# julesser/crocoddyl

Measured on AMD Instinct MI355X. Metric: FDDP iterations/sec + MPC solves/sec, Talos contact T=100, batch=1024, higher is better.
Workload: dtype f64

## Files before the change

### crocoddyl_amd/_abi.py

```python
import ctypes as C

ABI_VERSION = 3

FDDP_OK = 0
FDDP_ERR_INVALID_ARG = -1
FDDP_ERR_RUNTIME = -2
FDDP_ERR_UNSUPPORTED = -3
FDDP_ERR_NO_DEVICE = -4
FDDP_ERR_CALLBACK_ABORT = -5

STATUS_RUNNING, STATUS_CONVERGED, STATUS_REGMAX = 0, 1, 2

KNOT_LQR, KNOT_UNICYCLE, KNOT_EULER_DIFFLQR, KNOT_EULER_FREEFWD, KNOT_EULER_CONTACTFWD, KNOT_IMPULSEFWD = 1, 2, 3, 4, 5, 6
PARAM_HEADER = 4

Q_FX, Q_FU, Q_LXX, Q_LXU, Q_LUU, Q_LX, Q_LU, Q_XNEXT, Q_FS, Q_K, Q_KV = range(11)
Q_COST = 19
Q_VXX, Q_VX, Q_QXX, Q_QXU, Q_QUU, Q_QX, Q_QU = range(11, 18)
Q_QUU_INV = 18

SOLVER_FDDP, SOLVER_BOXFDDP = 0, 1

MB_W2, MB_W1, MB_X2, MB_X8, MB_S2 = range(5)
FWD_GENERIC, FWD_FAST, FWD_MB, FWD_MB2 = range(4)
# ... 83 lines not shown
    "get_x0": (C.c_int, [P, D]),
    "get_params": (C.c_int, [P, C.POINTER(Params)]),
    "get_xs": (C.c_int, [P, D, C.c_int]),
    "get_us": (C.c_int, [P, D, C.c_int]),
    "get_xs_try": (C.c_int, [P, D]),
    "get_us_try": (C.c_int, [P, D]),
    "set_debug": (C.c_int, [P, C.c_int]),
    "synchronize": (C.c_int, [P]),
    "get_stream": (C.c_int, [P, C.POINTER(P)]),
    "get_timing": (C.c_int, [P, D, C.POINTER(C.c_int64)]),
    "set_timing": (C.c_int, [P, C.c_int]),
    "device_bytes": (C.c_int64, [P]),
    "get_solver_kind": (C.c_int, [P, I32]),
    "set_callback": (C.c_int, [P, IterationCallback, C.c_void_p]),
    "get_line_search_info": (C.c_int, [P, I32, I32]),
    "get_kernel_info": (C.c_int, [P, I32]),
    "boxqp_default_params": (None, [C.POINTER(BoxQPParams)]),
    "boxqp_solve": (C.c_int, [C.c_int, C.c_int, C.c_int, D, D, D, D, D, C.POINTER(BoxQPParams), D, U64, U64, D, I32]),
}


def bind(lib, prefix, protos):
    for name, (res, args) in protos.items():
        fn = getattr(lib, prefix + name)
        fn.restype = res
        fn.argtypes = args


def dptr(a):
    if a is None:
# ... 3 lines not shown
```

### crocoddyl_amd/csrc/fddp_device.hpp

```cpp
#pragma once

#include <hip/hip_runtime.h>
#include <stdint.h>

#include "../../include/fddp_hip.h"

namespace fddp {

__host__ __device__ inline bool is_mb_kind(int kind) {
  return kind == FDDP_KNOT_EULER_FREEFWD || kind == FDDP_KNOT_EULER_CONTACTFWD || kind == FDDP_KNOT_IMPULSEFWD;
}

constexpr int kWave = 64;

struct ElemState {
  double cost;
  double cost_try;
  double stop;
  double xreg, ureg;
  double steplength;
  double dV, dVexp;
  double dg, dq, dv;
  double d0, d1;
  int32_t is_feasible, was_feasible;
  int32_t recalc;
  int32_t iter;
  int32_t status;
  int32_t active;
// ... 266 lines not shown
```

### crocoddyl_amd/csrc/fddp_hip.hip

```cpp
#define FDDP_TU_MAIN 1
#include <hip/hip_runtime.h>

#include <algorithm>
#include <cmath>
#include <cstdio>
#include <cstdlib>
#include <cstring>
#include <string>
#include <vector>

#include "../../include/fddp_hip.h"
#include "fddp_device.hpp"
#include "fddp_kernels.hpp"
#include "fast_path.hpp"
#include "bwd_mfma.hpp"
#include "ktab.hpp"
#include "launch_plan.hpp"

using namespace fddp;
using plan::block_doubles;
using plan::mb_block_check;

namespace fddp {
namespace ktab {
// ... 124 lines not shown
  o.mb_spill = env_int("FDDP_MB_SPILL", -1);
  o.fwd_mb_off = is0("FDDP_FWD_MB");
  o.fwd_mbw = env_int("FDDP_FWD_MBW", 0);
  if (const char* ew = env("FDDP_BWD_WAVES")) o.bwd_waves = ew[0] == '1' ? 1 : (ew[0] == '4' ? 4 : 8);
  o.bwd_generic = env("FDDP_BACKWARD") && std::strcmp(env("FDDP_BACKWARD"), "generic") == 0;
  o.fast_off = is0("FDDP_FAST");
  if (prev)
    o.ls_par = prev->ls_par;
  else if (env("CROCODDYL_AMD_LS_PAR"))
    o.ls_par = std::max(1, std::min(16, env_int("CROCODDYL_AMD_LS_PAR", 0)));
  return o;
}

}

struct fddp_handle_s {
  fddp_dims dims;
  int device = 0;
  int cus = 0;
  plan::LaunchPlan plan;
  int npar_alloc = 1;
  bool npar_chosen = false;
  hipStream_t stream = nullptr;
  std::vector<fddp_knot_desc> knots;
  int64_t n_params = 0;
  int64_t params_cap = 0;
  fddp_params prm;
  Dev D;
  std::vector<void*> allocs;
  double* staging = nullptr;
  int64_t staging_len = 0;
  double* d_out = nullptr;
  int* d_count = nullptr;
  int* h_count = nullptr;
  bool debug = false;
  double* dbg[7] = {nullptr, nullptr, nullptr, nullptr, nullptr, nullptr, nullptr};
  double* dqi = nullptr;
// ... 172 lines not shown
    KLAUNCH(ktab::backward_mfma(h->plan.var.bwd, dim3(D.B), h->stream, D, to_prm(h->prm), mode));
  else
    KLAUNCH(ktab::backward_generic(dim3(D.B), h->bwd_smem, h->stream, D, to_prm(h->prm), mode));
  return FDDP_OK;
}

static int ensure_par_slots(fddp_handle* h) {
  Dev& D = h->D;
  if (D.npar <= h->npar_alloc) return FDDP_OK;
  const int64_t B = D.B, K1 = D.T + 1, K0 = D.T, q = D.npar - 1;
  int rc;
  double* done = nullptr;
  if ((rc = dalloc(h, &D.pxs, q * B * K1 * D.sX)) || (rc = dalloc(h, &D.pus, q * B * K0 * D.sM)) ||
      (rc = dalloc(h, &D.pxnext, q * B * K0 * D.sX)) || (rc = dalloc(h, &D.pkcost, q * B * K1)) ||
      (rc = dalloc(h, &D.pdvp, q * B * K1)) || (rc = dalloc(h, &D.ptrial, B * D.npar * 4)) ||
      (rc = dalloc(h, &done, (B + 1) / 2)))
    return rc;
  D.ls_done = (int*)done;
  h->npar_alloc = D.npar;
  return FDDP_OK;
}

static void choose_npar(fddp_handle* h, const std::vector<ElemState>& st) {
  if (!h->plan.lds.npar_adapt || h->plan.lds.fast) return;
  const int na = h->prm.n_alphas;
  std::vector<int> t;
  t.reserve(st.size());
  for (const ElemState& s : st) {
    if (s.n_iter_run <= 0) continue;
    int k = na;
    for (int a = 0; a < na; ++a)
      if (s.steplength == h->prm.alphas[a]) {
        k = a + 1;
        break;
      }
    t.push_back(k);
  }
  if (t.empty()) return;
  const double S = h->plan.var.ls_slots;
  double best = 0.;
  int best_g = 1;
  for (int g : {1, 2, 4}) {
    double time = 0.;
    if (g == 1) {
      double w = 0.;
      int tmax = 0;
      for (int v : t) w += v, tmax = std::max(tmax, v);
      time = std::max(std::ceil(w / S), (double)tmax);
    } else {
      for (int k0 = 0; k0 < na; k0 += g) {
        const int slots = std::min(g, na - k0);
        double u = 0.;
        for (int v : t) u += v > k0 ? slots : 0;
        if (u > 0.) time += std::ceil(u / S);
      }
    }
    if (g == 1 || time < best) best = time, best_g = g;
  }
  h->D.npar = best_g;
  h->npar_chosen = true;
}

static int update_ls_order(fddp_handle* h, const std::vector<ElemState>& st) {
  Dev& D = h->D;
  const int B = D.B, na = h->prm.n_alphas;
  if (B < 2 || h->plan.lds.fast) return FDDP_OK;
  if (!D.ls_order) {
    double* p = nullptr;
    int rc;
    if ((rc = dalloc(h, &p, (B + 1) / 2))) return rc;
    D.ls_order = (const int*)p;
  }
  std::vector<int> key(B);
  for (int b = 0; b < B; ++b) {
    const ElemState& s = st[b];
    int k = 0;
    if (s.n_iter_run > 0) {
      k = na;
      for (int a = 0; a < na; ++a)
        if (s.steplength == h->prm.alphas[a]) {
          k = a + 1;
          break;
        }
    }
    key[b] = k;
  }
  h->h_order.resize(B);
  for (int b = 0; b < B; ++b) h->h_order[b] = b;
  std::stable_sort(h->h_order.begin(), h->h_order.end(), [&](int x, int y) { return key[x] > key[y]; });
  HIP_TRY(hipMemcpyAsync((void*)D.ls_order, h->h_order.data(), sizeof(int) * B, hipMemcpyHostToDevice, h->stream));
  return FDDP_OK;
}

int launch_forward(fddp_handle* h, int mode, double alpha, int* count) {
  Timed tm(h, 3);
  const Dev& D = h->D;
  if (!h->plan.lds.fast && mode == 0 && D.npar > 1) {
    int rc;
    if ((rc = ensure_par_slots(h))) return rc;
    const int na = h->prm.n_alphas, G = (na + D.npar - 1) / D.npar;
    h->ls_npar_last = D.npar;
    h->ls_launches_last = G;
    const int v = h->plan.var.fwd;
    for (int g = 0; g < G; ++g) {
      KLAUNCH(ktab::forward(v, dim3(D.B, D.npar), h->plan.lds.fwd_smem, h->stream, D, to_prm(h->prm), 2, 1., nullptr, h->plan.lds.pcap,
                            g));
      KLAUNCH(ktab::ls_select(dim3(D.B), h->stream, D, to_prm(h->prm), g, g == G - 1 ? 1 : 0, count));
    }
    return FDDP_OK;
  }
  if (mode == 0) {
// ... 98 lines not shown

int apply_knots(fddp_handle* h, const fddp_knot_desc* knots, const double* params, int64_t n_params) {
  Dev& D = h->D;
  const fddp_dims& d = h->dims;
  const int64_t K1 = (int64_t)d.T + 1;
  int rc;
  h->knots.assign(knots, knots + K1);
  plan::LaunchPlan& P = h->plan;
  P.ov = read_overrides(&P.ov);
  P.lds = plan::plan_lds(d, knots, params, n_params, P.ov);
  const plan::LdsPlan& L = P.lds;
  D.mbw = L.mbw;
  D.mbw_fwd = L.mbw_fwd;
  D.mbspill = L.mbspill;
  D.mbd = L.mbd;
  if (!(h->npar_chosen && L.has_mb && !P.ov.ls_par)) D.npar = L.npar;
  if (L.error) return fail(FDDP_ERR_INVALID_ARG, L.error);
  D.dxv_mbw = L.dxv_mbw;
  if (n_params > h->params_cap) {
    double* p = nullptr;
    if ((rc = dalloc(h, &p, n_params))) return rc;
    D.params = p;
    h->params_cap = n_params;
  }
  h->n_params = n_params;
  HIP_TRY(hipMemcpyAsync((void*)D.params, params, sizeof(double) * n_params, hipMemcpyHostToDevice, h->stream));
  if (!D.knots) {
    fddp_knot_desc* kd = nullptr;
    if ((rc = dalloc(h, (double**)&kd, (sizeof(fddp_knot_desc) * K1 + 7) / 8))) return rc;
    D.knots = kd;
  }
// ... 186 lines not shown
    return bail(fail(FDDP_ERR_RUNTIME, "hipHostMalloc"));

  std::vector<ElemState> st0(B);
  for (auto& s : st0) {
    std::memset(&s, 0, sizeof(s));
    s.xreg = NAN;
    s.ureg = NAN;
    s.steplength = 1.;
  }
  if (hipMemcpyAsync(D.st, st0.data(), sizeof(ElemState) * B, hipMemcpyHostToDevice, h->stream) != hipSuccess)
    return bail(fail(FDDP_ERR_RUNTIME, "upload state"));
  if ((rc = apply_knots(h, knots, params, n_params))) return bail(rc);
  if (const char* e = std::getenv("FDDP_STAMPS")) {
    if (e[0] == '1') {
      double* p2 = nullptr;
      if ((rc = dalloc(h, &p2, (int64_t)d.B * 140))) return bail(rc);
      D.stamps = (unsigned long long*)p2;
    }
  }
  if (hipStreamSynchronize(h->stream) != hipSuccess) return bail(fail(FDDP_ERR_RUNTIME, "sync after create"));
  *out = h;
  return FDDP_OK;
}

void fddp_destroy(fddp_handle* h) {
  if (!h) return;
  DeviceGuard g(h->device);
  if (h->stream) (void)hipStreamSynchronize(h->stream);
  if (h->D.stamps) {
    std::vector<unsigned long long> v((size_t)h->dims.B * 140);
    if (hipMemcpy(v.data(), h->D.stamps, v.size() * 8, hipMemcpyDeviceToHost) == hipSuccess) {
      const char* names[8] = {"p1_G", "p1_H", "p1_inv", "b1_dma", "p2_K", "p2_Vupd", "b2_p3", "b3_wait"};
      std::fprintf(stderr, "[fddp stamps] mean cycles per element (variant %d):\n", h->plan.var.bwd);
      for (int w = 0; w < h->plan.var.bwd % 10; ++w) {
        std::fprintf(stderr, "  wave %d:", w);
        for (int ph = 0; ph < 8; ++ph) {
          double s2 = 0;
          for (int b = 0; b < h->dims.B; ++b) s2 += (double)v[((size_t)b * 8 + w) * 8 + ph];
          std::fprintf(stderr, " %s=%.0f", names[ph], s2 / h->dims.B);
        }
        std::fprintf(stderr, "\n");
      }
      if (h->plan.lds.has_mb || h->plan.lds.fast) {
        const char* mn[5] = {"state", "params", "gains", "calc", "stores_checks"};
        std::fprintf(stderr, "[fddp stamps] %s rollout, wave 0's mean cycles per element (all trials):",
// ... 2 lines not shown
          double s2 = 0;
          for (int b = 0; b < h->dims.B; ++b) s2 += (double)v[(size_t)h->dims.B * 128 + (size_t)b * 8 + ph];
          std::fprintf(stderr, " %s=%.0f", mn[ph], s2 / h->dims.B);
        }
        std::fprintf(stderr, "\n");
      }
      {
        struct Ev {
          unsigned long long t;
          int d;
        };
        std::vector<std::pair<unsigned long long, std::vector<Ev>>> cus;
        std::vector<std::pair<unsigned long long, std::vector<Ev>>>* pc = &cus;
        unsigned long long t0 = ~0ull, t1 = 0;
        int n = 0;
        for (int b = 0; b < h->dims.B; ++b) {
          const unsigned long long* r = &v[(size_t)h->dims.B * 136 + (size_t)b * 4];
          if (r[0] == 0 || r[2] == 0) continue;
          const unsigned long long hw = r[1];
          const unsigned long long key = ((hw >> 32) << 16) | ((hw >> 8) & 0xff);
          size_t i = 0;
          while (i < pc->size() && (*pc)[i].first != key) ++i;
          if (i == pc->size()) pc->push_back({key, {}});
          (*pc)[i].second.push_back({r[0], 1});
          (*pc)[i].second.push_back({r[2], -1});
          t0 = std::min(t0, r[0]);
          t1 = std::max(t1, r[2]);
          ++n;
        }
        int most = 0;
        double area = 0.;
// ... 190 lines not shown
        if (out) std::copy(cbres.begin(), cbres.end(), out);
        return fail(FDDP_ERR_CALLBACK_ABORT, "fddp_solve: stopped by the iteration callback at iteration " +
                                                 std::to_string(it));
      }
    }
    if (it + 1 < maxiter) {
      HIP_TRY(hipMemcpyAsync(h->h_count, h->d_count, sizeof(int), hipMemcpyDeviceToHost, h->stream));
      HIP_TRY(hipStreamSynchronize(h->stream));
      if (*h->h_count == 0) break;
    }
  }
  if (out) {
    std::vector<ElemState> st;
    if ((rc = download_states(h, st))) return rc;
    for (int b = 0; b < D.B; ++b) fill_result(st[b], &out[b]);
    choose_npar(h, st);
    if ((rc = update_ls_order(h, st))) return rc;
  } else {
    HIP_TRY(hipStreamSynchronize(h->stream));
  }
  if (D.box_stats) {
    unsigned long long bs[4];
    HIP_TRY(hipMemcpy(bs, D.box_stats, sizeof(bs), hipMemcpyDeviceToHost));
    fprintf(stderr, "fddp box stats: %llu QPs, %.3f Newton iterations and %.3f inverses per QP\n", bs[0],
            bs[0] ? (double)bs[1] / bs[0] : 0., bs[0] ? (double)bs[2] / bs[0] : 0.);
  }
  return FDDP_OK;
}

int fddp_get_kernel_info(fddp_handle* h, int32_t out[8]) {
  if (!h || !out) return fail(FDDP_ERR_INVALID_ARG, "fddp_get_kernel_info: null argument");
  DeviceGuard g(h->device);
  out[0] = h->plan.var.mb;
  out[1] = h->plan.var.fwd;
  out[2] = h->plan.var.bwd;
  out[3] = h->D.mbspill;
  out[4] = (int32_t)h->plan.lds.mb_diff_smem;
  out[5] = (int32_t)(h->plan.lds.fast ? h->plan.lds.fwd_fast_smem : h->plan.lds.fwd_smem);
  out[6] = h->D.npar;
  out[7] = 0;
  return FDDP_OK;
}

int fddp_get_line_search_info(fddp_handle* h, int* group_size, int* launches) {
  if (!h) return fail(FDDP_ERR_INVALID_ARG, "fddp_get_line_search_info: null handle");
  if (group_size) *group_size = h->ls_npar_last;
  if (launches) *launches = h->ls_launches_last;
  return FDDP_OK;
}

int fddp_set_callback(fddp_handle* h, fddp_iteration_callback cb, void* user) {
  if (!h) return fail(FDDP_ERR_INVALID_ARG, "fddp_set_callback: null handle");
  if (h->in_solve) return fail(FDDP_ERR_INVALID_ARG, "fddp_set_callback: not from inside a callback");
  h->cb = cb;
  h->cb_user = cb ? user : nullptr;
  return FDDP_OK;
}

int fddp_get_results(fddp_handle* h, fddp_result* out) {
  if (!h || !out) return fail(FDDP_ERR_INVALID_ARG, "fddp_get_results: null");
  DeviceGuard g(h->device);
  std::vector<ElemState> st;
// ... 429 lines not shown
```

### crocoddyl_amd/csrc/fddp_kernels.hpp

```cpp
#pragma once

#include "fddp_device.hpp"
#include "box_qp.hpp"
#include "knots.hpp"

namespace fddp {


__device__ inline int64_t block_doubles_dev(int kind, int nx, int nu, const double* g = nullptr) {
  if (is_mb_kind(kind)) return (int64_t)g[3];
  if (kind == FDDP_KNOT_LQR) return FDDP_PARAM_HEADER + 2LL * nx * nx + 2LL * nx * nu + (int64_t)nu * nu + 2LL * nx + nu;
  if (kind == FDDP_KNOT_UNICYCLE) return FDDP_PARAM_HEADER;
  const int64_t nq = nx / 2;
  return FDDP_PARAM_HEADER + 2 * nq * nq + nq * nu + nq + (int64_t)nx * nx + (int64_t)nx * nu + (int64_t)nu * nu + nx +
         nu;
}

template <int NT>
__device__ __forceinline__ void state_diff_wg(const Dev& D, const double* x0, const double* x1, double* out,
                                              int first = 0) {
  const int n = D.n;
  if (D.nx == n) {
    for (int i = threadIdx.x; i < n; i += NT) out[i] = x1[i] - x0[i];
    return;
// ... 836 lines not shown
    s.iter += 1;
  }
}

#ifndef FDDP_FWD_WPE
#define FDDP_FWD_WPE 2
#endif
#ifndef FDDP_FWD_WPE_MB
#define FDDP_FWD_WPE_MB 3
#endif
template <int NT, bool FAST, bool MB = false, int MBW = FDDP_FWD_WPE_MB>
__global__ __launch_bounds__(NT) __attribute__((amdgpu_waves_per_eu(MB ? MBW : FAST ? FDDP_FWD_WPE : 1))) void forward_kernel(Dev D, Prm prm, int mode, double alpha1, int* active_count,
                                                     int64_t pcap, int group = 0) {
  const int b = D.ls_order ? D.ls_order[blockIdx.x] : (int)blockIdx.x;
  ElemState* st = D.st + b;
  if (mode != 1 && !st->active) return;
  const int slot = mode == 2 ? (int)blockIdx.y : 0;
  const int a2 = group * D.npar + slot;
  if (mode == 2 && (D.ls_done[b] || a2 >= prm.n_alphas)) return;
  extern __shared__ __attribute__((aligned(16))) double sm[];
  double* pl = sm;
  const double* cached = nullptr;
  double *xv, *uv, *xn, *red, *dxv = nullptr, *pa = nullptr, *pdyn = nullptr;
  int* flag;
  if (FAST) {
    xv = pl + pcap;
    uv = xv + D.sX;
    dxv = xv + D.sX + D.sM;
    xn = dxv + D.sN;
    pa = xn + D.sX;
    pdyn = pa + NT;
    red = pdyn + NT;
    flag = (int*)(red + 24);
  } else {
    xv = pl + pcap;
    uv = xv + D.sX;
    xn = uv + D.sM;
    red = xn + D.sX;
    flag = (int*)(red + 5 * (NT / kWave) + 8);
  }
  __shared__ ElemState ss;
  if (threadIdx.x == 0) ss = *st;
#ifdef FDDP_STAMPS_BUILD
  unsigned long long* rs = D.stamps && slot == 0 ? D.stamps + (int64_t)D.B * 136 + (int64_t)b * 4 : nullptr;
  if (rs && threadIdx.x == 0) {
    rs[0] = __builtin_amdgcn_s_memrealtime();
    rs[1] = (unsigned long long)(unsigned)__builtin_amdgcn_s_getreg(4 | (31 << 11)) |
            ((unsigned long long)(unsigned)__builtin_amdgcn_s_getreg(20 | (31 << 11)) << 32);
  }
#endif
  __syncthreads();
  int nwr = D.T + 1;
  double* const mbw = (double*)flag + 2 + (D.dxv_mbw ? 0 : 2 * D.sN);
  double* const dxv_ = D.dxv_mbw ? mbw + D.mbw_fwd - 2 * D.sN : (double*)flag + 2;
  auto trial = [&](double alpha, double& ct, double& dv) {
    if constexpr (FAST)
      return fwd_trial_fast<NT, true>(D, b, ss, alpha, xv, dxv, xn, pa, pdyn, red, flag, ct, dv, pl, pcap, cached);
    else
      return fwd_trial<NT, MB>(D, b, ss, alpha, xv, uv, xn, red, flag, ct, dv, pl, pcap, cached, mbw, dxv_, slot, &nwr);
  };
  bool accepted = false;
  const int na = mode == 0 ? prm.n_alphas : 1;
  for (int a = 0; a < na; ++a) {
    const double alpha = mode == 1 ? alpha1 : prm.alphas[mode == 2 ? a2 : a];
    double ct, dv;
    bool ok;
    [[clang::always_inline]] ok = trial(alpha, ct, dv);
    if (mode == 1) {
      if (threadIdx.x == 0) {
        st->fwd_fail = ok ? 0 : 1;
        st->cost_try = ct;
        st->dV = ss.cost - ct;
        st->dv = ok ? dv : 0.;
      }
      return;
    }
    if (mode == 2) {
      if (threadIdx.x == 0) {
        double* r = D.ptrial + ((int64_t)b * D.npar + slot) * 4;
        r[0] = ok ? 1. : 0.;
        r[1] = ct;
        r[2] = dv;
        r[3] = (double)nwr;
      }
      return;
    }
    ElemState s = ss;
    s.steplength = alpha;
    const bool acc = ok && ls_accept(prm, s, alpha, ct, dv);
    __syncthreads();
    if (threadIdx.x == 0) ss = s;
    __syncthreads();
    if (acc) {
      accepted = true;
      break;
    }
  }
  ElemState s = ss;
  ls_finish(prm, s, accepted);
#ifdef FDDP_STAMPS_BUILD
  if (rs && threadIdx.x == 0) rs[2] = __builtin_amdgcn_s_memrealtime();
#endif
  if (threadIdx.x == 0) {
    *st = s;
    if (s.active && active_count) atomicAdd(active_count, 1);
  }
}

template <int NT>
__global__ __launch_bounds__(NT) void ls_select_kernel(Dev D, Prm prm, int group, int last, int* active_count) {
  const int b = blockIdx.x, tid = threadIdx.x;
  ElemState* st = D.st + b;
  if (!st->active || D.ls_done[b]) {
    if (last && tid == 0) D.ls_done[b] = 0;
    return;
  }
  ElemState s = *st;
  int acc_slot = -1;
  bool exhausted = false;
  for (int p = 0; p < D.npar; ++p) {
    const int a = group * D.npar + p;
    if (a >= prm.n_alphas) {
      exhausted = true;
      break;
    }
    const double alpha = prm.alphas[a];
    s.steplength = alpha;
    const double* r = D.ptrial + ((int64_t)b * D.npar + p) * 4;
    if (r[0] == 0.) continue;
    if (ls_accept(prm, s, alpha, r[1], r[2])) {
      acc_slot = p;
      break;
    }
  }
  if (group * D.npar + D.npar >= prm.n_alphas) exhausted = true;
  auto copy_slot = [&](int p, int buf) {
    const TrialOut src(D, 0, p), dst(D, buf, 0);
    const int64_t K1 = (int64_t)D.ptrial[((int64_t)b * D.npar + p) * 4 + 3];
    const int64_t K0 = K1 < D.T ? K1 : D.T;
    for (int64_t i = tid; i < K1 * D.sX; i += NT) dst.xs[D.knot(b, 0) * D.sX + i] = src.xs[D.knot(b, 0) * D.sX + i];
    for (int64_t i = tid; i < K0 * D.sM; i += NT) dst.us[D.run(b, 0) * D.sM + i] = src.us[D.run(b, 0) * D.sM + i];
    for (int64_t i = tid; i < K0 * D.sX; i += NT)
      dst.xnext[D.run(b, 0) * D.sX + i] = src.xnext[D.run(b, 0) * D.sX + i];
    for (int64_t i = tid; i < K1; i += NT) dst.kcost[D.knot(b, 0) + i] = src.kcost[D.knot(b, 0) + i];
  };
  if (acc_slot < 0) {
    const int np = prm.n_alphas - group * D.npar < D.npar ? prm.n_alphas - group * D.npar : D.npar;
    for (int p = 1; p < np; ++p) copy_slot(p, 1 - s.cur);
    if (!exhausted) {
      if (tid == 0) *st = s;
      return;
    }
  } else if (acc_slot > 0) {
    copy_slot(acc_slot, s.cur);
  }
  ls_finish(prm, s, acc_slot >= 0);
  if (tid == 0) {
    *st = s;
    D.ls_done[b] = last ? 0 : 1;
    if (s.active && active_count) atomicAdd(active_count, 1);
  }
}

template <int NT>
__global__ __launch_bounds__(NT) void mpc_shift_kernel(Dev D) {
  const int b = blockIdx.x;
  ElemState* st = D.st + b;
  const int c = st->cur, o = 1 - c, T = D.T;
  const double* xs = D.xs[c] + D.knot(b, 0) * D.sX;
  double* xo = D.xs[o] + D.knot(b, 0) * D.sX;
  const double* us = D.us[c] + D.run(b, 0) * D.sM;
  double* uo = D.us[o] + D.run(b, 0) * D.sM;
  for (int64_t e = threadIdx.x; e < (int64_t)(T + 1) * D.sX; e += NT) {
    const int64_t t = e / D.sX, i = e % D.sX;
// ... 101 lines not shown
```

### crocoddyl_amd/csrc/launch_plan.hpp

```cpp
#ifndef CROCODDYL_AMD_LAUNCH_PLAN_HPP_
#define CROCODDYL_AMD_LAUNCH_PLAN_HPP_

#include <algorithm>
#include <cmath>
#include <cstdint>
#include <string>
#include <utility>
#include <vector>

#include "fddp_kernels.hpp"
#include "fast_path.hpp"
#include "ktab.hpp"
#include "multibody.hpp"

namespace fddp {
namespace plan {

constexpr int64_t kLdsTwoPerCu = 80 * 1024, kLdsFourPerCu = 40 * 1024;

struct Overrides {
  int mb_w1 = -1;
  int mb_nt = 0;
  int mb_spill = -1;
  int fwd_mb_off = 0;
// ... 19 lines not shown
  bool all_mb = false;
  bool has_icom = false;
  bool has_hmom = false;
  bool has_act = false;
  bool has_pris = false;
  int mb_nj = 0;
  int64_t mbw = 0, mbw_fwd = 0, mbd = 0;
  int mbspill = 0, dxv_mbw = 0;
  int64_t mb_all_lds = 0;
  size_t mb_diff_smem = 0;
  int64_t pcap = 0;
  size_t fwd_smem = 0, calc_smem = 0, cdiff_smem = 0, fused_smem = 0, fwd_fast_smem = 0;
  bool fast = false;
  int npar = 1;
  bool npar_adapt = false;
  bool uniform_nu = false;
  int ntl = 0, mtl = 0;
};

struct VariantPlan {
  int mb = -1;
  int fwd = 0;
  int bwd = 0;
  double ls_slots = 0.;
};

struct LaunchPlan {
  Overrides ov;
  LdsPlan lds;
  VariantPlan var;
// ... 272 lines not shown
          seen = seen || (q.nj == k.nj && q.njac == k.njac && q.nc == k.nc && q.nu == k.nu && q.nrows == k.nrows &&
                          q.vcols == k.vcols && q.act == k.act);
        if (!seen) shapes.push_back(k);
      }
    } else {
      p.all_mb = false;
      sz = block_doubles(knots[t].kind, d.nx, knots[t].nu);
    }
    pmax = std::max<int64_t>(pmax, sz);
  }
  p.mbw = p.has_mb ? pad2(fddp::mb::calc_work_doubles(mb_nj, mb_nc)) : 0;
  p.mbw_fwd = p.has_mb ? pad2(fddp::mb::calc_dense_doubles(mb_nj, mb_nc)) : 0;
  p.mb_nj = mb_nj;
  p.npar = ov.ls_par ? ov.ls_par : (p.has_mb && mb_nj >= 24 ? 4 : 1);
  p.npar_adapt = !ov.ls_par && p.has_mb;
  auto plan_doubles = [&](int spill) {
    int64_t mx = 0;
    for (const MbShape& q : shapes)
      mx = std::max<int64_t>(
          mx, pad2(fddp::mb::diff_layout(q.nj, q.njac, q.nc, q.vcols, q.nu, q.nrows, spill, q.act).total));
    return mx;
  };
  p.mb_all_lds = p.has_mb ? (plan_doubles(0) + pad2(mb_pmax)) * 8 : 0;
  p.mbspill = p.has_mb && !mb_act && !p.has_pris && ov.mb_spill != 0 && p.mb_all_lds > kLdsTwoPerCu
                  ? fddp::mb::diff_spill(mb_nj, mb_njac, mb_nc, mb_vcols, mb_nu, mb_nrows, mb_pmax, d.nu_max, mb_act)
                  : 0;
  p.mbd = p.has_mb ? plan_doubles(p.mbspill) : 0;
  p.mb_diff_smem = p.has_mb ? sizeof(double) * (p.mbd + pad2(mb_pmax)) : 0;
  const int64_t budget = (150 * 1024) / 8 - (2 * sX + sM + 2 * sN + 5 * (kNT / kWave) + 16) - p.mbw;
  p.pcap = pmax <= budget ? pad2(pmax) : (pad2(mb_pmax) <= budget ? pad2(mb_pmax) : 0);
// ... 66 lines not shown
      if (nw == 1 && !(ntl + mtl <= 4 && mtl == 1)) nw = 8;
      if (f.bwd_code[bwd_slot(nw)] < 0 && nw == 4) nw = 8;
      bwd = f.bwd_code[bwd_slot(nw)];
      const int occ = f.bwd_occ[bwd_slot(nw)], v4 = f.bwd_code[bwd_slot(4)], occ4 = f.bwd_occ[bwd_slot(4)];
      if (!ov.bwd_waves && bwd > 0 && mtl == 1 && v4 > 0 && f.cus > 0 && occ > 0 && occ4 > 0) {
        const int64_t r8 = (d.B + (int64_t)f.cus * occ - 1) / ((int64_t)f.cus * occ);
        const int64_t r4 = (d.B + (int64_t)f.cus * occ4 - 1) / ((int64_t)f.cus * occ4);
        if (1.2 * (double)r4 < (double)r8) bwd = v4;
      }
    }
  }
  v.bwd = bwd > 0 ? bwd : 0;
  return v;
}

}
}

#endif
```

### crocoddyl_amd/problem.py

```python
import ctypes as C
import math
import warnings

import numpy as np

from . import _abi
from ._lib import FDDPError, check, default_params, lib
from .host import HostProblem, HostSolverFDDP, is_host_model
from .models import ActionData, ActionModelAbstract


def pack_problem(running, terminal, B, cache=None):
    models = list(running) + [terminal]
    for m in models:
        if not isinstance(m, ActionModelAbstract) or m.kind is None:
            raise NotImplementedError(f"crocoddyl_amd: knot model {type(m).__name__} has no device implementation")
    offsets = {}
    pool = []
    pos = 0
    knots = []
    for m in models:
        key = id(m)
        if key not in offsets:
            if cache is not None:
# ... 687 lines not shown
    def get_timing(self):
        ms = np.zeros(4)
        cnt = np.zeros(4, dtype=np.int64)
        check(lib().fddp_get_timing(self._ptr, _abi.dptr(ms), cnt.ctypes.data_as(C.POINTER(C.c_int64))))
        names = ["calc", "calcDiff", "backward", "forward"]
        return {n: (float(ms[i]), int(cnt[i])) for i, n in enumerate(names)}

    def synchronize(self):
        check(lib().fddp_synchronize(self._ptr))

    def line_search_info(self):
        g, n = C.c_int32(), C.c_int32()
        check(lib().fddp_get_line_search_info(self._ptr, C.byref(g), C.byref(n)))
        return g.value, n.value


class SolverBoxFDDP(SolverFDDP):

    def __init__(self, problem):
        super().__init__(problem)
        check(lib().fddp_set_solver_kind(self._h.ptr, _abi.SOLVER_BOXFDDP))
        self._prm.th_stop = 5e-5
        self._push_params()

    @property
    def Quu_inv(self):
        p = self.problem
        return self._quantity(_abi.Q_QUU_INV, p.T, p.nu_max, p.nu_max, "both")
```

### include/crocoddyl_amd/solver_fddp_hip.hpp

```cpp
#ifndef CROCODDYL_AMD_SOLVER_FDDP_HIP_HPP_
#define CROCODDYL_AMD_SOLVER_FDDP_HIP_HPP_

#include <cmath>
#include <cstdio>
#include <exception>
#include <memory>
#include <stdexcept>
#include <string>
#include <vector>

#include "../fddp_hip.h"

namespace crocoddyl_amd {

struct Exception : std::runtime_error {
  explicit Exception(const std::string& m) : std::runtime_error(m) {}
};

inline void check(int rc, const char* what) {
  if (rc != FDDP_OK) throw Exception(std::string(what) + ": " + fddp_last_error());
}

typedef std::vector<double> VectorXd;

// ... 294 lines not shown
    check(fddp_expected_improvement(h_.get(), d.data()), "fddp_expected_improvement");
    return {d[0], d[1]};
  }
  double get_cost_try() const { return costs_try_.empty() ? 0. : costs_try_[0]; }
  const std::vector<double>& get_costs() const { return costs_; }
  const std::vector<double>& get_costs_try() const { return costs_try_; }
  const std::vector<int32_t>& get_step_status() const { return step_status_; }
  std::vector<VectorXd> get_K() const { return quantity(FDDP_Q_K, dims_.T, (size_t)dims_.nu_max * dims_.ndx); }
  std::vector<VectorXd> get_k() const { return quantity(FDDP_Q_KV, dims_.T, dims_.nu_max); }
  std::vector<VectorXd> get_fs() const { return quantity(FDDP_Q_FS, dims_.T + 1, dims_.ndx); }
  std::vector<VectorXd> get_Vxx() const { return quantity(FDDP_Q_VXX, dims_.T + 1, (size_t)dims_.ndx * dims_.ndx); }
  std::vector<VectorXd> get_Vx() const { return quantity(FDDP_Q_VX, dims_.T + 1, dims_.ndx); }
  std::vector<VectorXd> get_Quu() const { return quantity(FDDP_Q_QUU, dims_.T, (size_t)dims_.nu_max * dims_.nu_max); }
  std::vector<VectorXd> get_Qu() const { return quantity(FDDP_Q_QU, dims_.T, dims_.nu_max); }
  void set_debug(bool on) { check(fddp_set_debug(h_.get(), on ? 1 : 0), "fddp_set_debug"); }
  std::vector<VectorXd> get_xs_try() const {
    VectorXd a((size_t)dims_.B * (dims_.T + 1) * dims_.nx);
    check(fddp_get_xs_try(h_.get(), a.data()), "fddp_get_xs_try");
    std::vector<VectorXd> out;
    for (int t = 0; t <= dims_.T; ++t) out.push_back(VectorXd(a.begin() + t * dims_.nx, a.begin() + (t + 1) * dims_.nx));
    return out;
  }
  std::vector<VectorXd> get_us_try() const {
    VectorXd a((size_t)dims_.B * dims_.T * dims_.nu_max);
    check(fddp_get_us_try(h_.get(), a.data()), "fddp_get_us_try");
    std::vector<VectorXd> out;
    for (int t = 0; t < dims_.T; ++t)
      out.push_back(VectorXd(a.begin() + t * dims_.nu_max, a.begin() + (t + 1) * dims_.nu_max));
    return out;
  }
// ... 150 lines not shown
```

### include/fddp_hip.h

```cpp
#ifndef FDDP_HIP_H_
#define FDDP_HIP_H_

#include <stdint.h>

#ifdef __cplusplus
extern "C" {
#endif

#define FDDP_ABI_VERSION 3
int fddp_abi_version(void);

#define FDDP_OK 0
#define FDDP_ERR_INVALID_ARG (-1)
#define FDDP_ERR_RUNTIME (-2)
#define FDDP_ERR_UNSUPPORTED (-3)
#define FDDP_ERR_NO_DEVICE (-4)
#define FDDP_ERR_CALLBACK_ABORT (-5)

#define FDDP_STATUS_RUNNING 0
#define FDDP_STATUS_CONVERGED 1
#define FDDP_STATUS_REGMAX 2

#define FDDP_KNOT_LQR 1
#define FDDP_KNOT_UNICYCLE 2
// ... 68 lines not shown

int fddp_set_params(fddp_handle* h, const fddp_params* p);
int fddp_get_params(fddp_handle* h, fddp_params* p);

int fddp_set_candidate(fddp_handle* h, const double* xs, const double* us, int is_feasible);
int fddp_set_candidate_device(fddp_handle* h, const double* xs, const double* us, int is_feasible);

int fddp_solve(fddp_handle* h, int maxiter, int is_feasible, double reg_init, fddp_result* out);

typedef int (*fddp_iteration_callback)(void* user, int iter, const fddp_result* results, const int32_t* reported,
                                       int B);
int fddp_set_callback(fddp_handle* h, fddp_iteration_callback cb, void* user);

int fddp_get_line_search_info(fddp_handle* h, int* group_size, int* launches);

int fddp_get_kernel_info(fddp_handle* h, int32_t out[8]);

int fddp_get_results(fddp_handle* h, fddp_result* out);
int fddp_get_xs(fddp_handle* h, double* out, int on_device);
int fddp_get_us(fddp_handle* h, double* out, int on_device);

int fddp_problem_calc(fddp_handle* h, double* cost);
int fddp_problem_calc_diff(fddp_handle* h, double* cost);
int fddp_compute_direction(fddp_handle* h, int recalc, int32_t* status);
int fddp_calc_diff(fddp_handle* h, double* cost);
int fddp_backward_pass(fddp_handle* h, int32_t* status);
int fddp_forward_pass(fddp_handle* h, double step_length, double* cost_try, int32_t* status);
int fddp_update_expected_improvement(fddp_handle* h);
int fddp_try_step(fddp_handle* h, double alpha, double* dV, int32_t* status);
int fddp_expected_improvement(fddp_handle* h, double* d);
// ... 61 lines not shown
```

Before: 18480.

## Plan per-element line-search trial groups from previous accepted step counts

Adds a per-element line-search plan. The host predicts how many step-length trials each batch element will need, using the trial counts from the previous solve, and uploads those predictions. The forward pass then runs staged launches in which each element evaluates up to gmax alphas in parallel slots only while its prediction says it still needs them, followed by a serial finish launch. This targets idle slots and extra launches of uniform-group parallel search when elements need different numbers of trials. In exchange it adds host-side cost modelling, more launches per search, and wasted work when predictions are wrong. A public API to pin the prediction is also added.

```diff
diff --git a/crocoddyl_amd/_abi.py b/crocoddyl_amd/_abi.py
--- a/crocoddyl_amd/_abi.py
+++ b/crocoddyl_amd/_abi.py
@@ -121,6 +121,7 @@
     "get_solver_kind": (C.c_int, [P, I32]),
     "set_callback": (C.c_int, [P, IterationCallback, C.c_void_p]),
     "get_line_search_info": (C.c_int, [P, I32, I32]),
+    "set_line_search_plan": (C.c_int, [P, I32, C.c_int, C.c_int]),
     "get_kernel_info": (C.c_int, [P, I32]),
     "boxqp_default_params": (None, [C.POINTER(BoxQPParams)]),
     "boxqp_solve": (C.c_int, [C.c_int, C.c_int, C.c_int, D, D, D, D, D, C.POINTER(BoxQPParams), D, U64, U64, D, I32]),
diff --git a/crocoddyl_amd/csrc/fddp_device.hpp b/crocoddyl_amd/csrc/fddp_device.hpp
--- a/crocoddyl_amd/csrc/fddp_device.hpp
+++ b/crocoddyl_amd/csrc/fddp_device.hpp
@@ -12,6 +12,7 @@
 }
 
 constexpr int kWave = 64;
+constexpr int kLsMaxSlots = 4;
 
 struct ElemState {
   double cost;
diff --git a/crocoddyl_amd/csrc/fddp_hip.hip b/crocoddyl_amd/csrc/fddp_hip.hip
--- a/crocoddyl_amd/csrc/fddp_hip.hip
+++ b/crocoddyl_amd/csrc/fddp_hip.hip
@@ -162,6 +162,8 @@
 
 }
 
+constexpr int64_t kStampsPerElem = 136 + 4 * plan::kLsMaxSlots;
+
 struct fddp_handle_s {
   fddp_dims dims;
   int device = 0;
@@ -169,6 +171,11 @@
   plan::LaunchPlan plan;
   int npar_alloc = 1;
   bool npar_chosen = false;
+  bool ls_planned = false;
+  bool ls_pinned = false;
+  std::vector<int> h_pred;
+  int ls_tmax = 1;
+  std::vector<int32_t> ls_prev_trials;
   hipStream_t stream = nullptr;
   std::vector<fddp_knot_desc> knots;
   int64_t n_params = 0;
@@ -371,19 +378,18 @@
   if ((rc = dalloc(h, &D.pxs, q * B * K1 * D.sX)) || (rc = dalloc(h, &D.pus, q * B * K0 * D.sM)) ||
       (rc = dalloc(h, &D.pxnext, q * B * K0 * D.sX)) || (rc = dalloc(h, &D.pkcost, q * B * K1)) ||
       (rc = dalloc(h, &D.pdvp, q * B * K1)) || (rc = dalloc(h, &D.ptrial, B * D.npar * 4)) ||
-      (rc = dalloc(h, &done, (B + 1) / 2)))
+      (rc = dalloc(h, &done, (3 * B + 1) / 2)))
     return rc;
   D.ls_done = (int*)done;
   h->npar_alloc = D.npar;
   return FDDP_OK;
 }
 
-static void choose_npar(fddp_handle* h, const std::vector<ElemState>& st) {
-  if (!h->plan.lds.npar_adapt || h->plan.lds.fast) return;
+static std::vector<int32_t> last_trial_counts(const fddp_handle* h, const std::vector<ElemState>& st) {
   const int na = h->prm.n_alphas;
-  std::vector<int> t;
-  t.reserve(st.size());
-  for (const ElemState& s : st) {
+  std::vector<int32_t> t(st.size(), 0);
+  for (size_t b = 0; b < st.size(); ++b) {
+    const ElemState& s = st[b];
     if (s.n_iter_run <= 0) continue;
     int k = na;
     for (int a = 0; a < na; ++a)
@@ -391,36 +397,78 @@
         k = a + 1;
         break;
       }
-    t.push_back(k);
-  }
-  if (t.empty()) return;
+    t[b] = k;
+  }
+  return t;
+}
+
+static int install_ls_plan(fddp_handle* h, const int32_t* pred, int gmax) {
+  Dev& D = h->D;
+  const int B = D.B;
+  h->ls_planned = gmax > 1;
+  D.npar = std::max(1, gmax);
+  if (!h->ls_planned) return FDDP_OK;
+  int rc;
+  if ((rc = ensure_par_slots(h))) return rc;
+  h->h_pred.resize(B);
+  h->ls_tmax = 1;
+  for (int b = 0; b < B; ++b) {
+    h->h_pred[b] = std::max(1, (int)pred[b]);
+    h->ls_tmax = std::max(h->ls_tmax, h->h_pred[b]);
+  }
+  HIP_TRY(hipMemcpyAsync(D.ls_done + B, h->h_pred.data(), sizeof(int) * B, hipMemcpyHostToDevice, h->stream));
+  return FDDP_OK;
+}
+
+static int plan_next_search(fddp_handle* h, const std::vector<int32_t>& trials) {
+  if (!h->plan.lds.npar_adapt || h->plan.lds.fast || h->ls_pinned) return FDDP_OK;
+  bool any = false;
+  for (int32_t v : trials) any = any || v > 0;
+  if (!any) return FDDP_OK;
+  const int n = (int)trials.size(), na = h->prm.n_alphas;
   const double S = h->plan.var.ls_slots;
-  double best = 0.;
+  h->npar_chosen = true;
   int best_g = 1;
-  for (int g : {1, 2, 4}) {
-    double time = 0.;
-    if (g == 1) {
-      double w = 0.;
-      int tmax = 0;
-      for (int v : t) w += v, tmax = std::max(tmax, v);
-      time = std::max(std::ceil(w / S), (double)tmax);
-    } else {
-      for (int k0 = 0; k0 < na; k0 += g) {
-        const int slots = std::min(g, na - k0);
-        double u = 0.;
-        for (int v : t) u += v > k0 ? slots : 0;
-        if (u > 0.) time += std::ceil(u / S);
+  {
+    double best = 0.;
+    for (int g : {1, 2, 4}) {
+      double time = 0.;
+      if (g == 1) {
+        double w = 0.;
+        int tmax = 0;
+        for (int32_t v : trials)
+          if (v > 0) w += v, tmax = std::max(tmax, (int)v);
+        time = std::max(std::ceil(w / S), (double)tmax);
+      } else {
+        for (int k0 = 0; k0 < na; k0 += g) {
+          const int slots = std::min(g, na - k0);
+          double u = 0.;
+          for (int32_t v : trials) u += v > k0 ? slots : 0;
+          if (u > 0.) time += std::ceil(u / S);
+        }
       }
-    }
-    if (g == 1 || time < best) best = time, best_g = g;
-  }
+      if (g == 1 || time < best) best = time, best_g = g;
+    }
+  }
+  if (!h->plan.lds.ls_plan_adapt) {
+    h->ls_planned = false;
+    h->D.npar = best_g;
+    return FDDP_OK;
+  }
+  const plan::LsPlan p = plan::plan_line_search(trials.data(), n, na, S);
+  bool held = true;
+  if (p.plan && (int)h->ls_prev_trials.size() == n)
+    held = plan::ls_plan_time(h->ls_prev_trials.data(), trials.data(), n, na, p.gmax, S) < p.t_serial;
+  h->ls_prev_trials = trials;
+  if (p.plan && held) return install_ls_plan(h, trials.data(), p.gmax);
+  h->ls_planned = false;
   h->D.npar = best_g;
-  h->npar_chosen = true;
-}
-
-static int update_ls_order(fddp_handle* h, const std::vector<ElemState>& st) {
+  return FDDP_OK;
+}
+
+static int update_ls_order(fddp_handle* h, const std::vector<int32_t>& key) {
   Dev& D = h->D;
-  const int B = D.B, na = h->prm.n_alphas;
+  const int B = D.B;
   if (B < 2 || h->plan.lds.fast) return FDDP_OK;
   if (!D.ls_order) {
     double* p = nullptr;
@@ -428,20 +476,6 @@
     if ((rc = dalloc(h, &p, (B + 1) / 2))) return rc;
     D.ls_order = (const int*)p;
   }
-  std::vector<int> key(B);
-  for (int b = 0; b < B; ++b) {
-    const ElemState& s = st[b];
-    int k = 0;
-    if (s.n_iter_run > 0) {
-      k = na;
-      for (int a = 0; a < na; ++a)
-        if (s.steplength == h->prm.alphas[a]) {
-          k = a + 1;
-          break;
-        }
-    }
-    key[b] = k;
-  }
   h->h_order.resize(B);
   for (int b = 0; b < B; ++b) h->h_order[b] = b;
   std::stable_sort(h->h_order.begin(), h->h_order.end(), [&](int x, int y) { return key[x] > key[y]; });
@@ -452,6 +486,23 @@
 int launch_forward(fddp_handle* h, int mode, double alpha, int* count) {
   Timed tm(h, 3);
   const Dev& D = h->D;
+  if (D.stamps && mode == 0)
+    HIP_TRY(hipMemsetAsync(D.stamps + (size_t)D.B * 136, 0, sizeof(unsigned long long) * D.B * plan::kLsMaxSlots * 4, h->stream));
+  if (!h->plan.lds.fast && mode == 0 && D.npar > 1 && h->ls_planned) {
+    int rc;
+    if ((rc = ensure_par_slots(h))) return rc;
+    const int na = h->prm.n_alphas, K = plan::ls_group_stages(h->ls_tmax, na, D.npar);
+    h->ls_npar_last = std::min(D.npar, std::min(h->ls_tmax, na));
+    h->ls_launches_last = K + 1;
+    const int v = h->plan.var.fwd;
+    for (int k = 0; k < K; ++k) {
+      KLAUNCH(ktab::forward(v, dim3(D.B, D.npar), h->plan.lds.fwd_smem, h->stream, D, to_prm(h->prm), 3, 1., count, h->plan.lds.pcap,
+                            0));
+      KLAUNCH(ktab::ls_select(dim3(D.B), h->stream, D, to_prm(h->prm), k, 2, count));
+    }
+    KLAUNCH(ktab::forward(v, dim3(D.B), h->plan.lds.fwd_smem, h->stream, D, to_prm(h->prm), 3, 1., count, h->plan.lds.pcap, 1));
+    return FDDP_OK;
+  }
   if (!h->plan.lds.fast && mode == 0 && D.npar > 1) {
     int rc;
     if ((rc = ensure_par_slots(h))) return rc;
@@ -580,7 +631,10 @@
   D.mbw_fwd = L.mbw_fwd;
   D.mbspill = L.mbspill;
   D.mbd = L.mbd;
-  if (!(h->npar_chosen && L.has_mb && !P.ov.ls_par)) D.npar = L.npar;
+  if (!((h->npar_chosen && L.has_mb && !P.ov.ls_par) || h->ls_pinned)) {
+    D.npar = L.npar;
+    h->ls_planned = false;
+  }
   if (L.error) return fail(FDDP_ERR_INVALID_ARG, L.error);
   D.dxv_mbw = L.dxv_mbw;
   if (n_params > h->params_cap) {
@@ -797,7 +851,7 @@
   if (const char* e = std::getenv("FDDP_STAMPS")) {
     if (e[0] == '1') {
       double* p2 = nullptr;
-      if ((rc = dalloc(h, &p2, (int64_t)d.B * 140))) return bail(rc);
+      if ((rc = dalloc(h, &p2, (int64_t)d.B * kStampsPerElem))) return bail(rc);
       D.stamps = (unsigned long long*)p2;
     }
   }
@@ -811,7 +865,7 @@
   DeviceGuard g(h->device);
   if (h->stream) (void)hipStreamSynchronize(h->stream);
   if (h->D.stamps) {
-    std::vector<unsigned long long> v((size_t)h->dims.B * 140);
+    std::vector<unsigned long long> v((size_t)h->dims.B * kStampsPerElem);
     if (hipMemcpy(v.data(), h->D.stamps, v.size() * 8, hipMemcpyDeviceToHost) == hipSuccess) {
       const char* names[8] = {"p1_G", "p1_H", "p1_inv", "b1_dma", "p2_K", "p2_Vupd", "b2_p3", "b3_wait"};
       std::fprintf(stderr, "[fddp stamps] mean cycles per element (variant %d):\n", h->plan.var.bwd);
@@ -844,7 +898,7 @@
         std::vector<std::pair<unsigned long long, std::vector<Ev>>>* pc = &cus;
         unsigned long long t0 = ~0ull, t1 = 0;
         int n = 0;
-        for (int b = 0; b < h->dims.B; ++b) {
+        for (int b = 0; b < h->dims.B * plan::kLsMaxSlots; ++b) {
           const unsigned long long* r = &v[(size_t)h->dims.B * 136 + (size_t)b * 4];
           if (r[0] == 0 || r[2] == 0) continue;
           const unsigned long long hw = r[1];
@@ -1065,8 +1119,8 @@
     std::vector<ElemState> st;
     if ((rc = download_states(h, st))) return rc;
     for (int b = 0; b < D.B; ++b) fill_result(st[b], &out[b]);
-    choose_npar(h, st);
-    if ((rc = update_ls_order(h, st))) return rc;
+    const std::vector<int32_t> trials = last_trial_counts(h, st);
+    if ((rc = plan_next_search(h, trials)) || (rc = update_ls_order(h, trials))) return rc;
   } else {
     HIP_TRY(hipStreamSynchronize(h->stream));
   }
@@ -1097,6 +1151,31 @@
   if (!h) return fail(FDDP_ERR_INVALID_ARG, "fddp_get_line_search_info: null handle");
   if (group_size) *group_size = h->ls_npar_last;
   if (launches) *launches = h->ls_launches_last;
+  return FDDP_OK;
+}
+
+int fddp_set_line_search_plan(fddp_handle* h, const int32_t* pred, int n, int gmax) {
+  if (!h) return fail(FDDP_ERR_INVALID_ARG, "fddp_set_line_search_plan: null handle");
+  if (h->in_solve) return fail(FDDP_ERR_INVALID_ARG, "fddp_set_line_search_plan: not from inside a callback");
+  if (h->plan.ov.ls_par)
+    return fail(FDDP_ERR_INVALID_ARG, "fddp_set_line_search_plan: CROCODDYL_AMD_LS_PAR fixes this handle's trial groups");
+  DeviceGuard g(h->device);
+  if (n == 0) {
+    h->ls_pinned = false;
+    h->npar_chosen = false;
+    h->D.npar = h->plan.lds.npar;
+    h->ls_planned = false;
+    h->ls_prev_trials.clear();
+    return FDDP_OK;
+  }
+  if (!pred || n != h->D.B) return fail(FDDP_ERR_INVALID_ARG, "fddp_set_line_search_plan: pred must hold B entries");
+  if (gmax < 1 || gmax > plan::kLsMaxSlots)
+    return fail(FDDP_ERR_INVALID_ARG, "fddp_set_line_search_plan: gmax out of [1, 4]");
+  if (h->plan.lds.fast)
+    return fail(FDDP_ERR_UNSUPPORTED, "fddp_set_line_search_plan: the dense-knot fast path runs the serial search only");
+  const int rc = install_ls_plan(h, pred, gmax);
+  if (rc) return rc;
+  h->ls_pinned = true;
   return FDDP_OK;
 }
 
diff --git a/crocoddyl_amd/csrc/fddp_kernels.hpp b/crocoddyl_amd/csrc/fddp_kernels.hpp
--- a/crocoddyl_amd/csrc/fddp_kernels.hpp
+++ b/crocoddyl_amd/csrc/fddp_kernels.hpp
@@ -874,10 +874,37 @@
                                                      int64_t pcap, int group = 0) {
   const int b = D.ls_order ? D.ls_order[blockIdx.x] : (int)blockIdx.x;
   ElemState* st = D.st + b;
+  const int slot = mode >= 2 ? (int)blockIdx.y : 0;
+  bool single = mode == 2;
+  int a0 = 0;
+  if (mode == 3) {
+    const int done = D.ls_done[b];
+    int* const pred = D.ls_done + D.B;
+    int* const a0p = pred + D.B;
+    a0 = a0p[b];
+    if (group) {
+      if (blockIdx.y) return;
+      __syncthreads();
+      if (threadIdx.x == 0) {
+        D.ls_done[b] = 0;
+        a0p[b] = 0;
+      }
+      if (done) return;
+    } else {
+      if (done || !st->active) return;
+      int g = pred[b] - a0;
+      g = g < 1 ? 1 : (g > D.npar ? D.npar : g);
+      if (g > 1) {
+        single = true;
+        if (slot >= g) return;
+      } else {
+        if (blockIdx.y) return;
+      }
+    }
+  }
   if (mode != 1 && !st->active) return;
-  const int slot = mode == 2 ? (int)blockIdx.y : 0;
-  const int a2 = group * D.npar + slot;
-  if (mode == 2 && (D.ls_done[b] || a2 >= prm.n_alphas)) return;
+  const int a2 = mode == 3 ? a0 + slot : group * D.npar + slot;
+  if (single && ((mode == 2 && D.ls_done[b]) || a2 >= prm.n_alphas)) return;
   extern __shared__ __attribute__((aligned(16))) double sm[];
   double* pl = sm;
   const double* cached = nullptr;
@@ -902,7 +929,8 @@
   __shared__ ElemState ss;
   if (threadIdx.x == 0) ss = *st;
 #ifdef FDDP_STAMPS_BUILD
-  unsigned long long* rs = D.stamps && slot == 0 ? D.stamps + (int64_t)D.B * 136 + (int64_t)b * 4 : nullptr;
+  unsigned long long* rs =
+      D.stamps && slot < kLsMaxSlots ? D.stamps + (int64_t)D.B * 136 + ((int64_t)b * kLsMaxSlots + slot) * 4 : nullptr;
   if (rs && threadIdx.x == 0) {
     rs[0] = __builtin_amdgcn_s_memrealtime();
     rs[1] = (unsigned long long)(unsigned)__builtin_amdgcn_s_getreg(4 | (31 << 11)) |
@@ -920,9 +948,9 @@
       return fwd_trial<NT, MB>(D, b, ss, alpha, xv, uv, xn, red, flag, ct, dv, pl, pcap, cached, mbw, dxv_, slot, &nwr);
   };
   bool accepted = false;
-  const int na = mode == 0 ? prm.n_alphas : 1;
-  for (int a = 0; a < na; ++a) {
-    const double alpha = mode == 1 ? alpha1 : prm.alphas[mode == 2 ? a2 : a];
+  const int na = mode == 1 || single ? 1 : prm.n_alphas;
+  for (int a = single ? 0 : a0; a < na; ++a) {
+    const double alpha = mode == 1 ? alpha1 : prm.alphas[single ? a2 : a];
     double ct, dv;
     bool ok;
     [[clang::always_inline]] ok = trial(alpha, ct, dv);
@@ -935,7 +963,7 @@
       }
       return;
     }
-    if (mode == 2) {
+    if (single) {
       if (threadIdx.x == 0) {
         double* r = D.ptrial + ((int64_t)b * D.npar + slot) * 4;
         r[0] = ok ? 1. : 0.;
@@ -943,6 +971,9 @@
         r[2] = dv;
         r[3] = (double)nwr;
       }
+#ifdef FDDP_STAMPS_BUILD
+      if (rs && threadIdx.x == 0) rs[2] = __builtin_amdgcn_s_memrealtime();
+#endif
       return;
     }
     ElemState s = ss;
@@ -963,6 +994,7 @@
 #endif
   if (threadIdx.x == 0) {
     *st = s;
+    if (mode == 3 && !group) D.ls_done[b] = 1;
     if (s.active && active_count) atomicAdd(active_count, 1);
   }
 }
@@ -972,14 +1004,22 @@
   const int b = blockIdx.x, tid = threadIdx.x;
   ElemState* st = D.st + b;
   if (!st->active || D.ls_done[b]) {
-    if (last && tid == 0) D.ls_done[b] = 0;
+    if (last == 1 && tid == 0) D.ls_done[b] = 0;
     return;
   }
   ElemState s = *st;
+  int a0 = group * D.npar, g = D.npar;
+  const bool planned = last == 2;
+  if (planned) {
+    a0 = D.ls_done[2 * D.B + b];
+    g = D.ls_done[D.B + b] - a0;
+    g = g < 1 ? 1 : (g > D.npar ? D.npar : g);
+  }
+  __syncthreads();
   int acc_slot = -1;
   bool exhausted = false;
-  for (int p = 0; p < D.npar; ++p) {
-    const int a = group * D.npar + p;
+  for (int p = 0; p < g; ++p) {
+    const int a = a0 + p;
     if (a >= prm.n_alphas) {
       exhausted = true;
       break;
@@ -993,7 +1033,7 @@
       break;
     }
   }
-  if (group * D.npar + D.npar >= prm.n_alphas) exhausted = true;
+  if (a0 + g >= prm.n_alphas) exhausted = true;
   auto copy_slot = [&](int p, int buf) {
     const TrialOut src(D, 0, p), dst(D, buf, 0);
     const int64_t K1 = (int64_t)D.ptrial[((int64_t)b * D.npar + p) * 4 + 3];
@@ -1005,10 +1045,13 @@
     for (int64_t i = tid; i < K1; i += NT) dst.kcost[D.knot(b, 0) + i] = src.kcost[D.knot(b, 0) + i];
   };
   if (acc_slot < 0) {
-    const int np = prm.n_alphas - group * D.npar < D.npar ? prm.n_alphas - group * D.npar : D.npar;
+    const int np = prm.n_alphas - a0 < g ? prm.n_alphas - a0 : g;
     for (int p = 1; p < np; ++p) copy_slot(p, 1 - s.cur);
     if (!exhausted) {
-      if (tid == 0) *st = s;
+      if (tid == 0) {
+        *st = s;
+        if (planned) D.ls_done[2 * D.B + b] = a0 + g;
+      }
       return;
     }
   } else if (acc_slot > 0) {
@@ -1017,7 +1060,7 @@
   ls_finish(prm, s, acc_slot >= 0);
   if (tid == 0) {
     *st = s;
-    D.ls_done[b] = last ? 0 : 1;
+    D.ls_done[b] = last == 1 ? 0 : 1;
     if (s.active && active_count) atomicAdd(active_count, 1);
   }
 }
diff --git a/crocoddyl_amd/csrc/launch_plan.hpp b/crocoddyl_amd/csrc/launch_plan.hpp
--- a/crocoddyl_amd/csrc/launch_plan.hpp
+++ b/crocoddyl_amd/csrc/launch_plan.hpp
@@ -57,6 +57,7 @@
   bool fast = false;
   int npar = 1;
   bool npar_adapt = false;
+  bool ls_plan_adapt = false;
   bool uniform_nu = false;
   int ntl = 0, mtl = 0;
 };
@@ -359,6 +360,7 @@
   p.mb_nj = mb_nj;
   p.npar = ov.ls_par ? ov.ls_par : (p.has_mb && mb_nj >= 24 ? 4 : 1);
   p.npar_adapt = !ov.ls_par && p.has_mb;
+  p.ls_plan_adapt = p.npar_adapt && mb_nj >= 24;
   auto plan_doubles = [&](int spill) {
     int64_t mx = 0;
     for (const MbShape& q : shapes)
@@ -455,6 +457,85 @@
   return v;
 }
 
+using fddp::kLsMaxSlots;
+constexpr double kLsLaunchCost = 0.02;
+
+struct LsPlan {
+  bool plan = false;
+  int gmax = 1;
+  int stages = 0;
+  double t_serial = 0.;
+  double t_planned = 0.;
+};
+
+inline int ls_group_stages(int max_pred, int n_alphas, int gmax) {
+  const int t = std::max(1, std::min(max_pred, n_alphas));
+  return gmax > 1 ? (t + gmax - 1) / gmax : 0;
+}
+
+inline LsPlan plan_line_search(const int32_t* trials, int n, int n_alphas, double ls_slots) {
+  LsPlan r;
+  if (n <= 0 || n_alphas <= 0 || !(ls_slots >= 1.)) return r;
+  auto t_of = [&](int b) { return std::max(1, std::min((int)trials[b], n_alphas)); };
+  double w = 0.;
+  int tmax = 0, known = 0;
+  for (int b = 0; b < n; ++b) {
+    if (trials[b] > 0) ++known;
+    w += t_of(b);
+    tmax = std::max(tmax, t_of(b));
+  }
+  r.t_serial = r.t_planned = std::max(w / ls_slots, (double)tmax);
+  if (!known) return r;
+  for (int gmax = 2; gmax <= kLsMaxSlots; ++gmax) {
+    const int K = ls_group_stages(tmax, n_alphas, gmax);
+    double time = kLsLaunchCost * (K + 1);
+    for (int k = 0; k < K; ++k) {
+      const int a0 = k * gmax;
+      double u = 0.;
+      for (int b = 0; b < n; ++b)
+        if (t_of(b) > a0) u += std::min(t_of(b) - a0, gmax);
+      if (u > 0.) time += std::max(u / ls_slots, 1.);
+    }
+    if (time < r.t_planned) {
+      r.plan = true;
+      r.gmax = gmax;
+      r.stages = K;
+      r.t_planned = time;
+    }
+  }
+  return r;
+}
+
+inline double ls_plan_time(const int32_t* pred, const int32_t* actual, int n, int n_alphas, int gmax, double ls_slots) {
+  if (n <= 0 || n_alphas <= 0 || gmax < 2 || !(ls_slots >= 1.)) return 0.;
+  auto cl = [&](int v) { return std::max(1, std::min(v, n_alphas)); };
+  int pmax = 1;
+  for (int b = 0; b < n; ++b) pmax = std::max(pmax, cl(pred[b]));
+  const int K = ls_group_stages(pmax, n_alphas, gmax);
+  std::vector<int> a0(n, 0);
+  double time = kLsLaunchCost * (K + 1);
+  for (int k = 0; k <= K; ++k) {
+    double u = 0.;
+    int chain = 0;
+    for (int b = 0; b < n; ++b) {
+      const int t = cl(actual[b]);
+      if (a0[b] >= t) continue;
+      const int g = k == K ? 1 : std::max(1, std::min(cl(pred[b]) - a0[b], gmax));
+      if (g == 1) {
+        u += t - a0[b];
+        chain = std::max(chain, t - a0[b]);
+        a0[b] = t;
+      } else {
+        u += std::min(g, n_alphas - a0[b]);
+        chain = std::max(chain, 1);
+        a0[b] = a0[b] + g >= t ? t : a0[b] + g;
+      }
+    }
+    if (u > 0.) time += std::max(u / ls_slots, (double)chain);
+  }
+  return time;
+}
+
 }
 }
 
diff --git a/crocoddyl_amd/problem.py b/crocoddyl_amd/problem.py
--- a/crocoddyl_amd/problem.py
+++ b/crocoddyl_amd/problem.py
@@ -725,6 +725,13 @@
         check(lib().fddp_get_line_search_info(self._ptr, C.byref(g), C.byref(n)))
         return g.value, n.value
 
+    def set_line_search_plan(self, pred=None, gmax=4):
+        if pred is None:
+            check(lib().fddp_set_line_search_plan(self._ptr, None, 0, 0))
+            return
+        p = np.ascontiguousarray(pred, dtype=np.int32)
+        check(lib().fddp_set_line_search_plan(self._ptr, p.ctypes.data_as(_abi.I32), p.size, int(gmax)))
+
 
 class SolverBoxFDDP(SolverFDDP):
 
diff --git a/include/crocoddyl_amd/solver_fddp_hip.hpp b/include/crocoddyl_amd/solver_fddp_hip.hpp
--- a/include/crocoddyl_amd/solver_fddp_hip.hpp
+++ b/include/crocoddyl_amd/solver_fddp_hip.hpp
@@ -332,6 +332,10 @@
   std::vector<VectorXd> get_Quu() const { return quantity(FDDP_Q_QUU, dims_.T, (size_t)dims_.nu_max * dims_.nu_max); }
   std::vector<VectorXd> get_Qu() const { return quantity(FDDP_Q_QU, dims_.T, dims_.nu_max); }
   void set_debug(bool on) { check(fddp_set_debug(h_.get(), on ? 1 : 0), "fddp_set_debug"); }
+  void set_line_search_plan(const std::vector<int32_t>& pred, int gmax = 4) {
+    check(fddp_set_line_search_plan(h_.get(), pred.empty() ? nullptr : pred.data(), (int)pred.size(), gmax),
+          "fddp_set_line_search_plan");
+  }
   std::vector<VectorXd> get_xs_try() const {
     VectorXd a((size_t)dims_.B * (dims_.T + 1) * dims_.nx);
     check(fddp_get_xs_try(h_.get(), a.data()), "fddp_get_xs_try");
diff --git a/include/fddp_hip.h b/include/fddp_hip.h
--- a/include/fddp_hip.h
+++ b/include/fddp_hip.h
@@ -106,6 +106,8 @@
 
 int fddp_get_line_search_info(fddp_handle* h, int* group_size, int* launches);
 
+int fddp_set_line_search_plan(fddp_handle* h, const int32_t* pred, int n, int gmax);
+
 int fddp_get_kernel_info(fddp_handle* h, int32_t out[8]);
 
 int fddp_get_results(fddp_handle* h, fddp_result* out);
```

Result: faster. 19430, median of 6 (+5.2%).
